# run-house/kubetorch

Hardware: NVIDIA H100
Metric: parallel_map_arg_plus_result_GBps (higher is better)
Workload: dtype f32

## Files before the change

kubetorch_b200/csrc/ktb_mlp.cu:

```cuda
#include "ktb_common.cuh"

#include <cuda.h>
#include <algorithm>
#include <atomic>
#include <climits>
#include <cmath>
#include <mutex>

namespace ktb {

constexpr int kMlpBlockM = 128;
constexpr int kMlpBlockK = 64;
constexpr int kMlpWgmmaK = 16;
constexpr int kMlpStages = 4;
constexpr int kMlpConsumers = 256;
constexpr int kMlpThreads = kMlpConsumers + 32;
int g_mlp_chunk_rows = 16896;

__device__ __forceinline__ void tma_load_2d(void* smem_dst, const CUtensorMap* map, int c0, int c1, uint64_t* bar) {
  asm volatile(
      "cp.async.bulk.tensor.2d.shared::cluster.global.mbarrier::complete_tx::bytes [%0], [%1, {%3, %4}], [%2];" ::
          "r"(smem_u32(smem_dst)),
      "l"(map), "r"(smem_u32(bar)), "r"(c0), "r"(c1)
      : "memory");
}
__device__ __forceinline__ void prefetch_tensormap(const CUtensorMap* map) {
  asm volatile("prefetch.tensormap [%0];" ::"l"(map) : "memory");
}
__device__ __forceinline__ void mbar_arrive(uint64_t* bar) {
  asm volatile("mbarrier.arrive.shared::cta.b64 _, [%0];" ::"r"(smem_u32(bar)) : "memory");
}
__device__ __forceinline__ void wgmma_fence() { asm volatile("wgmma.fence.sync.aligned;" ::: "memory"); }
__device__ __forceinline__ void wgmma_commit() { asm volatile("wgmma.commit_group.sync.aligned;" ::: "memory"); }
__device__ __forceinline__ void wgmma_wait_all() { asm volatile("wgmma.wait_group.sync.aligned 0;" ::: "memory"); }

__device__ __forceinline__ uint64_t make_smem_desc_sw128(const void* smem_tile) {
  const uint32_t addr = smem_u32(smem_tile);
  uint64_t d = 0;
  d |= (uint64_t)((addr & 0x3FFFFu) >> 4);
  d |= (uint64_t)1 << 16;
  d |= (uint64_t)(1024u >> 4) << 32;
  d |= (uint64_t)1 << 62;
  return d;
}

template <int N>
struct Wgmma;
template <>
struct Wgmma<256> {
  __device__ __forceinline__ static void mma(float (&d)[128], uint64_t adesc, uint64_t bdesc, uint32_t scale_d) {
    asm volatile(
        "{\n"
        ".reg .pred p;\n"
        "setp.ne.b32 p, %130, 0;\n"
        "wgmma.mma_async.sync.aligned.m64n256k16.f32.bf16.bf16 "
        "{%0,%1,%2,%3,%4,%5,%6,%7,%8,%9,%10,%11,%12,%13,%14,%15,%16,%17,%18,%19,%20,%21,%22,%23,%24,%25,%26,%27,%28,%29,%30,%31,%32,%33,%34,%35,%36,%37,%38,%39,%40,%41,%42,%43,%44,%45,%46,%47,%48,%49,%50,%51,%52,%53,%54,%55,%56,%57,%58,%59,%60,%61,%62,%63,%64,%65,%66,%67,%68,%69,%70,%71,%72,%73,%74,%75,%76,%77,%78,%79,%80,%81,%82,%83,%84,%85,%86,%87,%88,%89,%90,%91,%92,%93,%94,%95,%96,%97,%98,%99,%100,%101,%102,%103,%104,%105,%106,%107,%108,%109,%110,%111,%112,%113,%114,%115,%116,%117,%118,%119,%120,%121,%122,%123,%124,%125,%126,%127}, "
        "%128, %129, p, 1, 1, 0, 0;\n"
        "}\n"
        : "+f"(d[0]), "+f"(d[1]), "+f"(d[2]), "+f"(d[3]), "+f"(d[4]), "+f"(d[5]), "+f"(d[6]), "+f"(d[7]), "+f"(d[8]), "+f"(d[9]), "+f"(d[10]), "+f"(d[11]), "+f"(d[12]), "+f"(d[13]), "+f"(d[14]), "+f"(d[15]), "+f"(d[16]), "+f"(d[17]), "+f"(d[18]), "+f"(d[19]), "+f"(d[20]), "+f"(d[21]), "+f"(d[22]), "+f"(d[23]), "+f"(d[24]), "+f"(d[25]), "+f"(d[26]), "+f"(d[27]), "+f"(d[28]), "+f"(d[29]), "+f"(d[30]), "+f"(d[31]), "+f"(d[32]), "+f"(d[33]), "+f"(d[34]), "+f"(d[35]), "+f"(d[36]), "+f"(d[37]), "+f"(d[38]), "+f"(d[39]), "+f"(d[40]), "+f"(d[41]), "+f"(d[42]), "+f"(d[43]), "+f"(d[44]), "+f"(d[45]), "+f"(d[46]), "+f"(d[47]), "+f"(d[48]), "+f"(d[49]), "+f"(d[50]), "+f"(d[51]), "+f"(d[52]), "+f"(d[53]), "+f"(d[54]), "+f"(d[55]), "+f"(d[56]), "+f"(d[57]), "+f"(d[58]), "+f"(d[59]), "+f"(d[60]), "+f"(d[61]), "+f"(d[62]), "+f"(d[63]), "+f"(d[64]), "+f"(d[65]), "+f"(d[66]), "+f"(d[67]), "+f"(d[68]), "+f"(d[69]), "+f"(d[70]), "+f"(d[71]), "+f"(d[72]), "+f"(d[73]), "+f"(d[74]), "+f"(d[75]), "+f"(d[76]), "+f"(d[77]), "+f"(d[78]), "+f"(d[79]), "+f"(d[80]), "+f"(d[81]), "+f"(d[82]), "+f"(d[83]), "+f"(d[84]), "+f"(d[85]), "+f"(d[86]), "+f"(d[87]), "+f"(d[88]), "+f"(d[89]), "+f"(d[90]), "+f"(d[91]), "+f"(d[92]), "+f"(d[93]), "+f"(d[94]), "+f"(d[95]), "+f"(d[96]), "+f"(d[97]), "+f"(d[98]), "+f"(d[99]), "+f"(d[100]), "+f"(d[101]), "+f"(d[102]), "+f"(d[103]), "+f"(d[104]), "+f"(d[105]), "+f"(d[106]), "+f"(d[107]), "+f"(d[108]), "+f"(d[109]), "+f"(d[110]), "+f"(d[111]), "+f"(d[112]), "+f"(d[113]), "+f"(d[114]), "+f"(d[115]), "+f"(d[116]), "+f"(d[117]), "+f"(d[118]), "+f"(d[119]), "+f"(d[120]), "+f"(d[121]), "+f"(d[122]), "+f"(d[123]), "+f"(d[124]), "+f"(d[125]), "+f"(d[126]), "+f"(d[127])
        : "l"(adesc), "l"(bdesc), "r"(scale_d));
  }
};

template <>
struct Wgmma<128> {
  __device__ __forceinline__ static void mma(float (&d)[64], uint64_t adesc, uint64_t bdesc, uint32_t scale_d) {
    asm volatile(
        "{\n"
        ".reg .pred p;\n"
        "setp.ne.b32 p, %66, 0;\n"
        "wgmma.mma_async.sync.aligned.m64n128k16.f32.bf16.bf16 "
        "{%0,%1,%2,%3,%4,%5,%6,%7,%8,%9,%10,%11,%12,%13,%14,%15,%16,%17,%18,%19,%20,%21,%22,%23,%24,%25,%26,%27,%28,%29,%30,%31,%32,%33,%34,%35,%36,%37,%38,%39,%40,%41,%42,%43,%44,%45,%46,%47,%48,%49,%50,%51,%52,%53,%54,%55,%56,%57,%58,%59,%60,%61,%62,%63}, "
        "%64, %65, p, 1, 1, 0, 0;\n"
        "}\n"
        : "+f"(d[0]), "+f"(d[1]), "+f"(d[2]), "+f"(d[3]), "+f"(d[4]), "+f"(d[5]), "+f"(d[6]), "+f"(d[7]), "+f"(d[8]), "+f"(d[9]), "+f"(d[10]), "+f"(d[11]), "+f"(d[12]), "+f"(d[13]), "+f"(d[14]), "+f"(d[15]), "+f"(d[16]), "+f"(d[17]), "+f"(d[18]), "+f"(d[19]), "+f"(d[20]), "+f"(d[21]), "+f"(d[22]), "+f"(d[23]), "+f"(d[24]), "+f"(d[25]), "+f"(d[26]), "+f"(d[27]), "+f"(d[28]), "+f"(d[29]), "+f"(d[30]), "+f"(d[31]), "+f"(d[32]), "+f"(d[33]), "+f"(d[34]), "+f"(d[35]), "+f"(d[36]), "+f"(d[37]), "+f"(d[38]), "+f"(d[39]), "+f"(d[40]), "+f"(d[41]), "+f"(d[42]), "+f"(d[43]), "+f"(d[44]), "+f"(d[45]), "+f"(d[46]), "+f"(d[47]), "+f"(d[48]), "+f"(d[49]), "+f"(d[50]), "+f"(d[51]), "+f"(d[52]), "+f"(d[53]), "+f"(d[54]), "+f"(d[55]), "+f"(d[56]), "+f"(d[57]), "+f"(d[58]), "+f"(d[59]), "+f"(d[60]), "+f"(d[61]), "+f"(d[62]), "+f"(d[63])
        : "l"(adesc), "l"(bdesc), "r"(scale_d));
  }
};

template <>
struct Wgmma<64> {
  __device__ __forceinline__ static void mma(float (&d)[32], uint64_t adesc, uint64_t bdesc, uint32_t scale_d) {
    asm volatile(
        "{\n"
        ".reg .pred p;\n"
        "setp.ne.b32 p, %34, 0;\n"
        "wgmma.mma_async.sync.aligned.m64n64k16.f32.bf16.bf16 "
        "{%0,%1,%2,%3,%4,%5,%6,%7,%8,%9,%10,%11,%12,%13,%14,%15,%16,%17,%18,%19,%20,%21,%22,%23,%24,%25,%26,%27,%28,%29,%30,%31}, "
        "%32, %33, p, 1, 1, 0, 0;\n"
        "}\n"
        : "+f"(d[0]), "+f"(d[1]), "+f"(d[2]), "+f"(d[3]), "+f"(d[4]), "+f"(d[5]), "+f"(d[6]), "+f"(d[7]), "+f"(d[8]), "+f"(d[9]), "+f"(d[10]), "+f"(d[11]), "+f"(d[12]), "+f"(d[13]), "+f"(d[14]), "+f"(d[15]), "+f"(d[16]), "+f"(d[17]), "+f"(d[18]), "+f"(d[19]), "+f"(d[20]), "+f"(d[21]), "+f"(d[22]), "+f"(d[23]), "+f"(d[24]), "+f"(d[25]), "+f"(d[26]), "+f"(d[27]), "+f"(d[28]), "+f"(d[29]), "+f"(d[30]), "+f"(d[31])
        : "l"(adesc), "l"(bdesc), "r"(scale_d));
  }
};
template <int BLOCK_N, int STAGES>
struct MlpSmem {
  static constexpr int kABytes = kMlpBlockM * kMlpBlockK * 2;
  static constexpr int kBBytes = BLOCK_N * kMlpBlockK * 2;
  static constexpr int kStageBytes = kABytes + kBBytes;
  static constexpr int kBarrierOff = STAGES * kStageBytes;
  static constexpr int kTotal = kBarrierOff + 2 * STAGES * 8 + 1024 ;
};

template <int BLOCK_N, int STAGES>
__device__ __forceinline__ bool mlp_tile_mainloop(const CUtensorMap* map_a, const CUtensorMap* map_b, int K, int m0,
                                                  int n0, float (&acc)[BLOCK_N / 2]) {
  using S = MlpSmem<BLOCK_N, STAGES>;
  extern __shared__ uint8_t smem_raw[];
  uint8_t* smem = reinterpret_cast<uint8_t*>((reinterpret_cast<uintptr_t>(smem_raw) + 1023) & ~(uintptr_t)1023);
  uint64_t* full = reinterpret_cast<uint64_t*>(smem + S::kBarrierOff);
  uint64_t* empty = full + STAGES;

  const int warp = threadIdx.x >> 5;
  const int lane = threadIdx.x & 31;
  const int num_kb = K / kMlpBlockK;

  if (threadIdx.x == 0) {
#pragma unroll
    for (int s = 0; s < STAGES; ++s) {
      mbar_init(&full[s], 1);
      mbar_init(&empty[s], kMlpConsumers);
    }
    fence_barrier_init();
  }
  __syncthreads();

  if (warp == kMlpConsumers / 32) {
    if (lane == 0) {
      prefetch_tensormap(map_a);
      prefetch_tensormap(map_b);
      for (int kb = 0; kb < num_kb; ++kb) {
        const int s = kb % STAGES;
        mbar_wait(&empty[s], ((kb / STAGES) & 1) ^ 1);
        uint8_t* a_dst = smem + (size_t)s * S::kStageBytes;
        mbar_expect_tx(&full[s], S::kStageBytes);
        tma_load_2d(a_dst, map_a, kb * kMlpBlockK, m0, &full[s]);
        tma_load_2d(a_dst + S::kABytes, map_b, kb * kMlpBlockK, n0, &full[s]);
      }
    }
    return false;
  }

  const int wg = warp >> 2;
#pragma unroll
  for (int i = 0; i < BLOCK_N / 2; ++i) acc[i] = 0.f;
  for (int kb = 0; kb < num_kb; ++kb) {
    const int s = kb % STAGES;
    mbar_wait(&full[s], (kb / STAGES) & 1);
    const uint8_t* a_src = smem + (size_t)s * S::kStageBytes + wg * 64 * 128;
    const uint64_t adesc = make_smem_desc_sw128(a_src);
    const uint64_t bdesc = make_smem_desc_sw128(smem + (size_t)s * S::kStageBytes + S::kABytes);
    wgmma_fence();
#pragma unroll
    for (int k = 0; k < kMlpBlockK / kMlpWgmmaK; ++k) {
      Wgmma<BLOCK_N>::mma(acc, adesc + (uint64_t)(2 * k), bdesc + (uint64_t)(2 * k), (uint32_t)((kb | k) != 0));
    }
    wgmma_commit();
    wgmma_wait_all();
    mbar_arrive(&empty[s]);
  }
  return true;
}

__device__ __forceinline__ bool argmax_before(float v, int col, float best, int best_col) {
  const bool v_nan = v != v, best_nan = best != best;
  if (v_nan || best_nan) return v_nan && (!best_nan || col < best_col);
  return v > best || (v == best && col < best_col);
}

__device__ __forceinline__ uint4 philox4x32_10(uint4 c, uint2 k) {
#pragma unroll
  for (int i = 0; i < 10; ++i) {
    const uint32_t hi0 = __umulhi(0xD2511F53u, c.x), lo0 = 0xD2511F53u * c.x;
    const uint32_t hi1 = __umulhi(0xCD9E8D57u, c.z), lo1 = 0xCD9E8D57u * c.z;
    c = make_uint4(hi1 ^ c.y ^ k.x, lo1, hi0 ^ c.w ^ k.y, lo0);
    k.x += 0x9E3779B9u;
    k.y += 0xBB67AE85u;
  }
  return c;
}

__device__ __forceinline__ float gumbel_of(uint32_t x) {
  const float u = (float)(2u * (x >> 9) + 1u) * 5.9604644775390625e-8f;
  return -logf(-logf(u));
}

__device__ __forceinline__ void layer_pair(float a0, float a1, float a2, float a3, const __nv_bfloat16* bias, int col,
                                           int n_valid, int relu, __nv_bfloat162& y0, __nv_bfloat162& y1) {
  float v[4] = {a0, a1, a2, a3};
  if (bias != nullptr) {
#pragma unroll
    for (int c = 0; c < 2; ++c) {
      if (col + c < n_valid) {
        const float b = __bfloat162float(bias[col + c]);
        v[c] += b;
        v[2 + c] += b;
      }
    }
  }
  if (relu) {
#pragma unroll
    for (int q = 0; q < 4; ++q) v[q] = fmaxf(v[q], 0.f);
  }
  y0 = __floats2bfloat162_rn(v[0], v[1]);
  y1 = __floats2bfloat162_rn(v[2], v[3]);
}

template <int BLOCK_N>
__device__ __forceinline__ void sample_epilogue(const float (&acc)[BLOCK_N / 2], const __nv_bfloat16* bias, int col0,
                                                int n_valid, int relu, int row, bool st0, bool st1, int64_t* actions,
                                                float* log_probs, uint64_t seed, uint64_t row_base) {
  float mx[2] = {-INFINITY, -INFINITY};
  __nv_bfloat162 y[BLOCK_N / 4];
#pragma unroll
  for (int j = 0; j < BLOCK_N / 8; ++j) {
    const int col = col0 + 8 * j;
    if (col >= n_valid) continue;
    layer_pair(acc[4 * j], acc[4 * j + 1], acc[4 * j + 2], acc[4 * j + 3], bias, col, n_valid, relu, y[2 * j],
               y[2 * j + 1]);
#pragma unroll
    for (int q = 0; q < 4; ++q) {
      const float v = q & 1 ? __high2float(y[2 * j + (q >> 1)]) : __low2float(y[2 * j + (q >> 1)]);
      if (col + (q & 1) < n_valid && v > mx[q >> 1]) mx[q >> 1] = v;
    }
  }
#pragma unroll
  for (int h = 0; h < 2; ++h) {
#pragma unroll
    for (int m = 1; m <= 2; m <<= 1) {
      const float o = __shfl_xor_sync(0xffffffffu, mx[h], m);
      if (o > mx[h]) mx[h] = o;
    }
  }
  const uint2 key = make_uint2((uint32_t)seed, (uint32_t)(seed >> 32));
  float best[2] = {-INFINITY, -INFINITY}, best_y[2] = {0.f, 0.f}, sum[2] = {0.f, 0.f};
  int best_col[2] = {INT_MAX, INT_MAX};
#pragma unroll
  for (int j = 0; j < BLOCK_N / 8; ++j) {
    const int col = col0 + 8 * j;
    if (col >= n_valid) continue;
#pragma unroll
    for (int h = 0; h < 2; ++h) {
      const uint64_t i = row_base + (uint64_t)(row + 8 * h);
      const uint4 x = philox4x32_10(make_uint4((uint32_t)i, (uint32_t)(i >> 32), (uint32_t)col >> 1, 0u), key);
#pragma unroll
      for (int c = 0; c < 2; ++c) {
        if (col + c >= n_valid) continue;
        const float v = c ? __high2float(y[2 * j + h]) : __low2float(y[2 * j + h]);
        const float s = v + gumbel_of(c ? x.y : x.x);
        if (argmax_before(s, col + c, best[h], best_col[h])) {
          best[h] = s;
          best_col[h] = col + c;
          best_y[h] = v;
        }
        sum[h] += v == mx[h] ? 1.f : expf(v - mx[h]);
      }
    }
  }
#pragma unroll
  for (int h = 0; h < 2; ++h) {
#pragma unroll
    for (int m = 1; m <= 2; m <<= 1) {
      const float ov = __shfl_xor_sync(0xffffffffu, best[h], m);
      const int oc = __shfl_xor_sync(0xffffffffu, best_col[h], m);
      const float oy = __shfl_xor_sync(0xffffffffu, best_y[h], m);
      sum[h] += __shfl_xor_sync(0xffffffffu, sum[h], m);
      if (argmax_before(ov, oc, best[h], best_col[h])) {
        best[h] = ov;
        best_col[h] = oc;
        best_y[h] = oy;
      }
    }
  }
  if ((threadIdx.x & 3) == 0) {
    if (st0) {
      actions[row] = best_col[0];
      log_probs[row] = best_y[0] - mx[0] - logf(sum[0]);
    }
    if (st1) {
      actions[row + 8] = best_col[1];
      log_probs[row + 8] = best_y[1] - mx[1] - logf(sum[1]);
    }
  }
}

template <int BLOCK_N, int STAGES>
__device__ __forceinline__ void gaussian_epilogue(const float (&acc)[BLOCK_N / 2], const __nv_bfloat16* bias, int col0,
                                                  int n_valid, int relu, int row, bool st0, bool st1,
                                                  const float* log_std, float* actions, float* log_probs,
                                                  uint64_t seed, uint64_t row_base) {
  asm volatile("" : "+l"(seed), "+l"(row_base), "+l"(bias), "+r"(col0), "+r"(n_valid), "+r"(row));
  using S = MlpSmem<BLOCK_N, STAGES>;
  static_assert(BLOCK_N / 64 <= STAGES, "each warp's bf16 pairs fill its 16 A rows of BLOCK_N / 64 stages");
  extern __shared__ uint8_t smem_raw[];
  uint8_t* smem = reinterpret_cast<uint8_t*>((reinterpret_cast<uintptr_t>(smem_raw) + 1023) & ~(uintptr_t)1023);
  uint8_t* mine = smem + (threadIdx.x >> 5) * 16 * 128 + (threadIdx.x & 31) * 4;
  auto slot = [&](int w) { return reinterpret_cast<__nv_bfloat162*>(mine + (w >> 4) * S::kStageBytes + (w & 15) * 128); };
#pragma unroll
  for (int j = 0; j < BLOCK_N / 8; ++j) {
    const int col = col0 + 8 * j;
    if (col >= n_valid) continue;
    layer_pair(acc[4 * j], acc[4 * j + 1], acc[4 * j + 2], acc[4 * j + 3], bias, col, n_valid, relu, *slot(2 * j),
               *slot(2 * j + 1));
  }
  const uint2 key = make_uint2((uint32_t)seed, (uint32_t)(seed >> 32));
  const bool pairs = (n_valid & 1) == 0 && ((uintptr_t)actions & 7) == 0;
  float sum[2] = {0.f, 0.f};
#pragma unroll 1
  for (int j = 0; j < BLOCK_N / 8; ++j) {
    const int col = col0 + 8 * j;
    if (col >= n_valid) break;
    const __nv_bfloat162 y[2] = {*slot(2 * j), *slot(2 * j + 1)};
    const bool has1 = col + 1 < n_valid;
    const float ls[2] = {log_std[col], has1 ? log_std[col + 1] : 0.f};
    const float sg[2] = {expf(ls[0]), expf(ls[1])};
#pragma unroll
    for (int h = 0; h < 2; ++h) {
      const uint64_t i = row_base + (uint64_t)(row + 8 * h);
      const uint4 x = philox4x32_10(make_uint4((uint32_t)i, (uint32_t)(i >> 32), (uint32_t)col >> 1, 1u), key);
      float a[2];
#pragma unroll
      for (int c = 0; c < 2; ++c) {
        const float u = (float)(2u * ((c ? x.y : x.x) >> 9) + 1u) * 5.9604644775390625e-8f;
        const float z = normcdfinvf(u);
        a[c] = __fadd_rn(c ? __high2float(y[h]) : __low2float(y[h]), __fmul_rn(sg[c], z));
        if (c == 0 || has1) sum[h] += 0.5f * z * z + ls[c];
      }
      if (!(h ? st1 : st0)) continue;
      float* p = actions + (size_t)(row + 8 * h) * n_valid + col;
      if (pairs) {
        *reinterpret_cast<float2*>(p) = make_float2(a[0], a[1]);
      } else {
        p[0] = a[0];
        if (has1) p[1] = a[1];
      }
    }
  }
#pragma unroll
  for (int h = 0; h < 2; ++h) {
#pragma unroll
    for (int m = 1; m <= 2; m <<= 1) sum[h] += __shfl_xor_sync(0xffffffffu, sum[h], m);
  }
  if ((threadIdx.x & 3) == 0) {
    const float c = (float)n_valid * 0.918938533204672742f;
    if (st0) log_probs[row] = -sum[0] - c;
    if (st1) log_probs[row + 8] = -sum[1] - c;
  }
}

template <int BLOCK_N, int STAGES>
__global__ void __launch_bounds__(kMlpThreads, 1)
    mlp_layer_wgmma_kernel(const __grid_constant__ CUtensorMap map_a, const __grid_constant__ CUtensorMap map_b,
                           const __nv_bfloat16* __restrict__ bias, __nv_bfloat16* __restrict__ C,
                           int64_t* __restrict__ actions, float* __restrict__ log_probs, uint64_t seed,
                           uint64_t row_base, const float* __restrict__ log_std, float* __restrict__ gauss_actions,
                           int ldc, int n_valid, int K, int rows, int relu) {
  const int n0 = blockIdx.x * BLOCK_N;
  const int m0 = blockIdx.y * kMlpBlockM;
  const int lane = threadIdx.x & 31;
  const int col0 = n0 + 2 * (lane & 3);
  float acc[BLOCK_N / 2];
  if (!mlp_tile_mainloop<BLOCK_N, STAGES>(&map_a, &map_b, K, m0, n0, acc)) return;
  const int warp = threadIdx.x >> 5;
  const int wg = warp >> 2;

  const int row = m0 + wg * 64 + (warp & 3) * 16 + (lane >> 2);
  const bool st0 = row < rows, st1 = row + 8 < rows;
  if (log_std != nullptr) {
    gaussian_epilogue<BLOCK_N, STAGES>(acc, bias, col0, n_valid, relu, row, st0, st1, log_std, gauss_actions,
                                       log_probs, seed, row_base);
    return;
  }
  if (log_probs != nullptr) {
    sample_epilogue<BLOCK_N>(acc, bias, col0, n_valid, relu, row, st0, st1, actions, log_probs, seed, row_base);
    return;
  }
  const bool pairs = C != nullptr && (ldc & 1) == 0 && ((uintptr_t)C & 3) == 0;
  if (pairs && actions == nullptr && n0 + BLOCK_N <= n_valid) {
    __nv_bfloat16* p0 = C + (size_t)row * ldc + col0;
    __nv_bfloat16* p1 = p0 + (size_t)8 * ldc;
#pragma unroll
    for (int j = 0; j < BLOCK_N / 8; ++j) {
      __nv_bfloat162 y0, y1;
      layer_pair(acc[4 * j], acc[4 * j + 1], acc[4 * j + 2], acc[4 * j + 3], bias, col0 + 8 * j, n_valid, relu, y0, y1);
      if (st0) *reinterpret_cast<__nv_bfloat162*>(p0 + 8 * j) = y0;
      if (st1) *reinterpret_cast<__nv_bfloat162*>(p1 + 8 * j) = y1;
    }
    return;
  }
  float best[2] = {-INFINITY, -INFINITY};
  int best_col[2] = {INT_MAX, INT_MAX};
#pragma unroll
  for (int j = 0; j < BLOCK_N / 8; ++j) {
    const int col = col0 + 8 * j;
    __nv_bfloat162 y0, y1;
    layer_pair(acc[4 * j], acc[4 * j + 1], acc[4 * j + 2], acc[4 * j + 3], bias, col, n_valid, relu, y0, y1);
    if (C != nullptr) {
      __nv_bfloat16* p0 = C + (size_t)row * ldc + col;
      __nv_bfloat16* p1 = p0 + (size_t)8 * ldc;
      if (pairs && col + 1 < n_valid) {
        if (st0) *reinterpret_cast<__nv_bfloat162*>(p0) = y0;
        if (st1) *reinterpret_cast<__nv_bfloat162*>(p1) = y1;
      } else {
        if (st0 && col < n_valid) p0[0] = y0.x;
        if (st1 && col < n_valid) p1[0] = y1.x;
        if (st0 && col + 1 < n_valid) p0[1] = y0.y;
        if (st1 && col + 1 < n_valid) p1[1] = y1.y;
      }
    }
    if (actions != nullptr) {
      const float r[4] = {__low2float(y0), __high2float(y0), __low2float(y1), __high2float(y1)};
#pragma unroll
      for (int q = 0; q < 4; ++q) {
        const int h = q >> 1, c = col + (q & 1);
        if (c < n_valid && argmax_before(r[q], c, best[h], best_col[h])) {
          best[h] = r[q];
          best_col[h] = c;
        }
      }
    }
  }
  if (actions != nullptr) {
#pragma unroll
    for (int h = 0; h < 2; ++h) {
#pragma unroll
      for (int m = 1; m <= 2; m <<= 1) {
        const float ov = __shfl_xor_sync(0xffffffffu, best[h], m);
        const int oc = __shfl_xor_sync(0xffffffffu, best_col[h], m);
        if (argmax_before(ov, oc, best[h], best_col[h])) {
          best[h] = ov;
          best_col[h] = oc;
        }
      }
    }
    if ((lane & 3) == 0) {
      if (st0) actions[row] = best_col[0];
      if (st1) actions[row + 8] = best_col[1];
    }
  }
}

typedef CUresult (*PFN_tensorMapEncodeTiled)(CUtensorMap*, CUtensorMapDataType, cuuint32_t, void*, const cuuint64_t*,
                                             const cuuint64_t*, const cuuint32_t*, const cuuint32_t*,
                                             CUtensorMapInterleave, CUtensorMapSwizzle, CUtensorMapL2promotion,
                                             CUtensorMapFloatOOBfill);
static PFN_tensorMapEncodeTiled g_encode = nullptr;
static std::once_flag g_encode_once;

static int get_encoder() {
  std::call_once(g_encode_once, [] {
    void* fn = nullptr;
    cudaDriverEntryPointQueryResult qres;
    if (cudaGetDriverEntryPoint("cuTensorMapEncodeTiled", &fn, cudaEnableDefault, &qres) == cudaSuccess &&
        qres == cudaDriverEntryPointSuccess)
      g_encode = reinterpret_cast<PFN_tensorMapEncodeTiled>(fn);
  });
  KTB_REQUIRE(g_encode != nullptr, KTB_ERR_CUDA, "cuTensorMapEncodeTiled is not available from the driver");
  return KTB_OK;
}

static int encode_map(CUtensorMap* map, const void* base, uint64_t rows, uint64_t cols, uint32_t box_rows);

static int make_map(CUtensorMap* map, const void* base, uint64_t rows, uint64_t cols, uint32_t box_rows) {
  struct Key {
    const void* base;
    uint64_t rows, cols;
    uint32_t box;
    bool operator==(const Key& o) const { return base == o.base && rows == o.rows && cols == o.cols && box == o.box; }
  };
  struct Slot {
    Key key;
    CUtensorMap map;
    bool used = false;
  };
  constexpr int kSlots = 64;
  thread_local Slot cache[kSlots];
  const Key k{base, rows, cols, box_rows};
  const size_t h = ((uintptr_t)base >> 8) * 0x9E3779B97F4A7C15ull + rows * 31 + cols * 7 + box_rows;
  Slot& s = cache[h % kSlots];
  if (s.used && s.key == k) {
    *map = s.map;
    return KTB_OK;
  }
  int rc = encode_map(map, base, rows, cols, box_rows);
  if (rc) return rc;
  s.key = k;
  s.map = *map;
  s.used = true;
  return KTB_OK;
}

static int encode_map(CUtensorMap* map, const void* base, uint64_t rows, uint64_t cols, uint32_t box_rows) {
  cuuint64_t gdim[2] = {cols, rows};
  cuuint64_t gstride[1] = {cols * 2};
  cuuint32_t box[2] = {(cuuint32_t)kMlpBlockK, box_rows};
  cuuint32_t estr[2] = {1, 1};
  CUresult r = g_encode(map, CU_TENSOR_MAP_DATA_TYPE_BFLOAT16, 2, const_cast<void*>(base), gdim, gstride, box, estr,
                        CU_TENSOR_MAP_INTERLEAVE_NONE, CU_TENSOR_MAP_SWIZZLE_128B, CU_TENSOR_MAP_L2_PROMOTION_L2_256B,
                        CU_TENSOR_MAP_FLOAT_OOB_FILL_NONE);
  KTB_REQUIRE(r == CUDA_SUCCESS, KTB_ERR_CUDA, "cuTensorMapEncodeTiled failed with CUresult %d", (int)r);
  return KTB_OK;
}

template <typename KernelT>
static int ensure_smem_attr(KernelT kfn, int smem_bytes, std::atomic<unsigned>& done_mask, int dev) {
  if (dev >= 0 && dev < 32 && (done_mask.load(std::memory_order_acquire) & (1u << dev))) return KTB_OK;
  cudaError_t e = cudaFuncSetAttribute(kfn, cudaFuncAttributeMaxDynamicSharedMemorySize, smem_bytes);
  if (e != cudaSuccess) {
    set_error("cudaFuncSetAttribute(max dynamic shared memory = %d) failed: %s", smem_bytes, cudaGetErrorString(e));
    return KTB_ERR_CUDA;
  }
  if (dev >= 0 && dev < 32) done_mask.fetch_or(1u << dev, std::memory_order_release);
  return KTB_OK;
}

template <int BLOCK_N>
static int launch_layer(int dev, const void* A, const void* B, const void* bias, void* C, int64_t* actions,
                        float* log_probs, uint64_t seed, uint64_t row_base, const float* log_std, float* gauss_actions,
                        size_t M, int N, int K, int ldc, bool relu, cudaStream_t stream) {
  using S = MlpSmem<BLOCK_N, kMlpStages>;
  static_assert(S::kTotal <= 232448, "the TMA ring must fit the 227 KiB a block may own");
  CUtensorMap ma, mb;
  int rc = make_map(&ma, A, M, (uint64_t)K, kMlpBlockM);
  if (rc) return rc;
  rc = make_map(&mb, B, (uint64_t)N, (uint64_t)K, BLOCK_N);
  if (rc) return rc;
  auto kfn = mlp_layer_wgmma_kernel<BLOCK_N, kMlpStages>;
  static std::atomic<unsigned> attr_done{0};
  rc = ensure_smem_attr(kfn, S::kTotal, attr_done, dev);
  if (rc) return rc;
  dim3 grid((unsigned)((N + BLOCK_N - 1) / BLOCK_N), (unsigned)((M + kMlpBlockM - 1) / kMlpBlockM));
  kfn<<<grid, kMlpThreads, S::kTotal, stream>>>(ma, mb, static_cast<const __nv_bfloat16*>(bias),
                                                static_cast<__nv_bfloat16*>(C), actions, log_probs, seed, row_base,
                                                log_std, gauss_actions, ldc, N, K, (int)M, relu);
  KTB_CK(cudaGetLastError());
  return KTB_OK;
}

struct MlpParams {
  const void *W1, *b1, *W2, *b2, *W3, *b3;
  void* logits;
  int64_t* actions;
  float* log_probs = nullptr;
  uint64_t seed = 0, row_base = 0;
  const float* log_std = nullptr;
  float* gauss_actions = nullptr;
};

static int mlp_hidden(int dev, const void* A, const void* W, const void* b, void* H, size_t rows, int d_hidden, int K,
                      cudaStream_t st) {
  return launch_layer<256>(dev, A, W, b, H, nullptr, nullptr, 0, 0, nullptr, nullptr, rows, d_hidden, K, d_hidden,
                           true, st);
}

static int mlp_head(int dev, const MlpParams& p, const void* h2, size_t r0, size_t rows, int d_hidden, int d_out,
                    cudaStream_t st) {
  void* y = p.logits ? static_cast<__nv_bfloat16*>(p.logits) + r0 * d_out : nullptr;
  int64_t* act = p.actions ? p.actions + r0 : nullptr;
  float* lp = p.log_probs ? p.log_probs + r0 : nullptr;
  float* ga = p.gauss_actions ? p.gauss_actions + r0 * d_out : nullptr;
  const uint64_t rb = p.row_base + r0;
  if (d_out <= 64)
    return launch_layer<64>(dev, h2, p.W3, p.b3, y, act, lp, p.seed, rb, p.log_std, ga, rows, d_out, d_hidden, d_out,
                            false, st);
  if (d_out <= 128)
    return launch_layer<128>(dev, h2, p.W3, p.b3, y, act, lp, p.seed, rb, p.log_std, ga, rows, d_out, d_hidden, d_out,
                             false, st);
  return launch_layer<256>(dev, h2, p.W3, p.b3, y, act, lp, p.seed, rb, p.log_std, ga, rows, d_out, d_hidden, d_out,
                           false, st);
}

static int mlp_check(const char* fn, size_t M, int d_in, int d_hidden, int d_out, const MlpParams& p, const void* obs,
                     const void* scratch, const void* stage) {
  KTB_REQUIRE(d_in > 0 && d_in % kMlpBlockK == 0, KTB_ERR_ARG, "%s: d_in=%d must be a multiple of 64", fn, d_in);
  KTB_REQUIRE(d_hidden > 0 && d_hidden % 256 == 0, KTB_ERR_ARG, "%s: d_hidden=%d must be a multiple of 256", fn,
              d_hidden);
  if (M > 0) {
    KTB_REQUIRE(p.logits || p.actions || p.log_std, KTB_ERR_ARG, "%s: logits and actions are both null", fn);
    if (p.log_std) {
      KTB_REQUIRE(p.gauss_actions && p.log_probs && !p.logits && !p.actions, KTB_ERR_ARG,
                  "%s: the Gaussian head needs fp32 actions and log_probs, and stores nothing else", fn);
      KTB_REQUIRE((((uintptr_t)p.log_std | (uintptr_t)p.gauss_actions) & 3) == 0, KTB_ERR_ARG,
                  "%s: log_std and actions must be 4-byte aligned", fn);
    }
    KTB_REQUIRE(d_out >= 1, KTB_ERR_ARG, "%s: d_out=%d must be positive", fn, d_out);
    KTB_REQUIRE(d_out <= 256, KTB_ERR_UNSUPPORTED, "%s: d_out=%d (heads up to 256 wide)", fn, d_out);
    KTB_REQUIRE((((uintptr_t)p.logits | (uintptr_t)p.b1 | (uintptr_t)p.b2 | (uintptr_t)p.b3) & 1) == 0, KTB_ERR_ARG,
                "%s: logits and biases must be 2-byte aligned", fn);
    KTB_REQUIRE(((uintptr_t)p.actions & 7) == 0, KTB_ERR_ARG, "%s: actions must be 8-byte aligned", fn);
    KTB_REQUIRE(((uintptr_t)p.log_probs & 3) == 0, KTB_ERR_ARG, "%s: log_probs must be 4-byte aligned", fn);
  }
  KTB_REQUIRE((((uintptr_t)obs | (uintptr_t)p.W1 | (uintptr_t)p.W2 | (uintptr_t)p.W3 | (uintptr_t)scratch |
                (uintptr_t)stage) & 15) == 0,
              KTB_ERR_ARG, "%s: obs, weights, scratch and stage must be 16-byte aligned", fn);
  return KTB_OK;
}
}

using namespace ktb;

extern "C" {

size_t ktb_mlp_scratch_bytes(size_t M, int d_hidden) {
  const size_t rows = std::min<size_t>(M, (size_t)g_mlp_chunk_rows);
  return 2 * rows * (size_t)d_hidden * 2;
}

size_t ktb_mlp_stage_bytes(size_t M, int d_in) {
  const size_t rows = std::min<size_t>(M, (size_t)g_mlp_chunk_rows);
  return 2 * rows * (size_t)d_in * 2;
}

int g_mlp_stage_ce = 0;

static int mlp_run(const char* fn, int dev, const void* obs, size_t M, int d_in, int d_hidden, int d_out,
                   const MlpParams& p, void* scratch, void* stage, uintptr_t stream) {
  int rc = require_device(dev);
  if (rc) return rc;
  if (M == 0) return KTB_OK;
  KTB_REQUIRE(obs && p.W1 && p.W2 && p.W3 && scratch, KTB_ERR_ARG, "%s: null argument", fn);
  rc = mlp_check(fn, M, d_in, d_hidden, d_out, p, obs, scratch, stage);
  if (rc) return rc;
  KTB_REQUIRE(g_mlp_chunk_rows % kMlpBlockM == 0 && g_mlp_chunk_rows > 0, KTB_ERR_ARG, "%s: bad chunk rows", fn);
  rc = get_encoder();
  if (rc) return rc;
  KTB_GUARD(dev);
  DeviceInfo* di = device_info(dev);
  cudaStream_t st = reinterpret_cast<cudaStream_t>(stream);
  cudaStream_t side = di->stream_exec;
  const size_t chunk = std::min<size_t>(M, (size_t)g_mlp_chunk_rows);
  __nv_bfloat16* h1 = static_cast<__nv_bfloat16*>(scratch);
  __nv_bfloat16* h2 = h1 + chunk * (size_t)d_hidden;
  const __nv_bfloat16* x = static_cast<const __nv_bfloat16*>(obs);
  __nv_bfloat16* stg = static_cast<__nv_bfloat16*>(stage);
  const MapParams ident = make_params(1, 0);
  cudaEvent_t evs[5] = {nullptr, nullptr, nullptr, nullptr, nullptr};
  struct EvGuard {
    cudaEvent_t* e;
    ~EvGuard() {
      for (int i = 0; i < 5; ++i)
        if (e[i]) cudaEventDestroy(e[i]);
    }
  } ev_guard{evs};
  static std::mutex side_mu[kMaxDevices];
  std::unique_lock<std::mutex> side_lock;
  if (stg) {
    side_lock = std::unique_lock<std::mutex>(side_mu[dev]);
    for (int i = 0; i < 5; ++i) KTB_CK(cudaEventCreateWithFlags(&evs[i], cudaEventDisableTiming));
    KTB_CK(cudaEventRecord(evs[0], st));
    KTB_CK(cudaStreamWaitEvent(side, evs[0], 0));
  }
  size_t c = 0;
  for (size_t r0 = 0; r0 < M; r0 += chunk, ++c) {
    const size_t rows = std::min(chunk, M - r0);
    const __nv_bfloat16* a1 = x + r0 * d_in;
    if (stg) {
      const int b = (int)(c & 1);
      __nv_bfloat16* dstb = stg + (size_t)b * chunk * d_in;
      if (c >= 2) KTB_CK(cudaStreamWaitEvent(side, evs[3 + b], 0));
      if (g_mlp_stage_ce) {
        KTB_CK(cudaMemcpyAsync(dstb, a1, rows * (size_t)d_in * 2, cudaMemcpyDefault, side));
      } else {
        rc = launch_map(dev, KTB_OP_IDENTITY, KTB_U8, a1, dstb, rows * (size_t)d_in * 2, ident, KTB_VARIANT_AUTO, side);
        if (rc) return rc;
      }
      KTB_CK(cudaEventRecord(evs[1 + b], side));
      KTB_CK(cudaStreamWaitEvent(st, evs[1 + b], 0));
      a1 = dstb;
    }
    rc = mlp_hidden(dev, a1, p.W1, p.b1, h1, rows, d_hidden, d_in, st);
    if (rc) return rc;
    if (stg) KTB_CK(cudaEventRecord(evs[3 + (int)(c & 1)], st));
    rc = mlp_hidden(dev, h1, p.W2, p.b2, h2, rows, d_hidden, d_hidden, st);
    if (rc) return rc;
    rc = mlp_head(dev, p, h2, r0, rows, d_hidden, d_out, st);
    if (rc) return rc;
  }
  return KTB_OK;
}

namespace ktb {
__global__ void mlp_wait_ready_kernel(const unsigned long long* ready, unsigned long long seq, unsigned int* status) {
  if (threadIdx.x == 0) (void)spin_until(ready, seq, status);
}
__global__ void mlp_ack_kernel(unsigned long long* ack, unsigned long long seq) {
  if (threadIdx.x == 0) {
    __threadfence_system();
    st_release_sys(ack, seq);
  }
}
}

static int mlp_pushed_run(const char* fn, int dev, const void* stage_local, size_t stage_stride, size_t M, int d_in,
                          int d_hidden, int d_out, const MlpParams& p, void* scratch, void* ctrl_local,
                          void* ctrl_root_peer, int rank, size_t chunk_rows, unsigned long long seq, uintptr_t stream) {
  int rc = require_device(dev);
  if (rc) return rc;
  KTB_REQUIRE(stage_local && ctrl_local && ctrl_root_peer && p.W1 && p.W2 && p.W3 && scratch, KTB_ERR_ARG,
              "%s: null argument", fn);
  KTB_REQUIRE(rank >= 0 && rank < 16 && seq > 0, KTB_ERR_ARG, "%s: bad rank/seq", fn);
  KTB_REQUIRE(M % kMlpBlockM == 0, KTB_ERR_ARG, "%s: M=%zu must be a multiple of %d", fn, M, kMlpBlockM);
  KTB_REQUIRE(chunk_rows > 0 && chunk_rows % kMlpBlockM == 0, KTB_ERR_ARG,
              "%s: chunk_rows=%zu must be a positive multiple of %d", fn, chunk_rows, kMlpBlockM);
  rc = mlp_check(fn, M, d_in, d_hidden, d_out, p, stage_local, scratch, nullptr);
  if (rc) return rc;
  const size_t n_chunks = (M + chunk_rows - 1) / chunk_rows;
  KTB_REQUIRE(n_chunks <= KTB_PUSH_MAX_CHUNKS, KTB_ERR_ARG, "%s: %zu chunks exceed %d", fn, n_chunks,
              KTB_PUSH_MAX_CHUNKS);
  KTB_REQUIRE(M * (size_t)d_in * 2 <= stage_stride, KTB_ERR_ARG, "%s: shard exceeds stage_stride", fn);
  rc = get_encoder();
  if (rc) return rc;
  KTB_GUARD(dev);
  cudaStream_t st = reinterpret_cast<cudaStream_t>(stream);
  uint8_t* cl = static_cast<uint8_t*>(ctrl_local);
  const unsigned long long* ready = reinterpret_cast<const unsigned long long*>(cl + KTB_CTRL_READY);
  unsigned int* status = reinterpret_cast<unsigned int*>(cl + KTB_CTRL_STATUS);
  unsigned long long* ack =
      reinterpret_cast<unsigned long long*>(static_cast<uint8_t*>(ctrl_root_peer) + KTB_CTRL_ACK) + rank;
  const __nv_bfloat16* x =
      reinterpret_cast<const __nv_bfloat16*>(static_cast<const uint8_t*>(stage_local) + (size_t)(seq & 1) * stage_stride);
  __nv_bfloat16* h1 = static_cast<__nv_bfloat16*>(scratch);
  __nv_bfloat16* h2 = h1 + std::min(chunk_rows, M) * (size_t)d_hidden;
  size_t c = 0;
  for (size_t r0 = 0; r0 < M; r0 += chunk_rows, ++c) {
    const size_t rows = std::min(chunk_rows, M - r0);
    mlp_wait_ready_kernel<<<1, 32, 0, st>>>(ready + c, seq, status);
    KTB_CK(cudaGetLastError());
    const __nv_bfloat16* a1 = x + r0 * d_in;
    rc = mlp_hidden(dev, a1, p.W1, p.b1, h1, rows, d_hidden, d_in, st);
    if (rc) return rc;
    rc = mlp_hidden(dev, h1, p.W2, p.b2, h2, rows, d_hidden, d_hidden, st);
    if (rc) return rc;
    rc = mlp_head(dev, p, h2, r0, rows, d_hidden, d_out, st);
    if (rc) return rc;
  }
  mlp_ack_kernel<<<1, 32, 0, st>>>(ack, seq);
  KTB_CK(cudaGetLastError());
  return KTB_OK;
}

int ktb_mlp_bf16_pushed(int dev, const void* stage_local, size_t stage_stride, size_t M, int d_in, int d_hidden, int d_out,
                        const void* W1, const void* W2, const void* W3, void* logits, void* scratch, void* ctrl_local,
                        void* ctrl_root_peer, int rank, size_t chunk_rows, unsigned long long seq, uintptr_t stream) {
  const char* fn = "ktb_mlp_bf16_pushed";
  int rc = require_device(dev);
  if (rc) return rc;
  KTB_REQUIRE(logits || M == 0, KTB_ERR_ARG, "%s: null argument", fn);
  KTB_REQUIRE(d_out == 64, KTB_ERR_UNSUPPORTED, "%s: d_out=%d (the 64-wide head)", fn, d_out);
  const MlpParams p{W1, nullptr, W2, nullptr, W3, nullptr, logits, nullptr};
  return mlp_pushed_run(fn, dev, stage_local, stage_stride, M, d_in, d_hidden, d_out, p, scratch, ctrl_local,
                        ctrl_root_peer, rank, chunk_rows, seq, stream);
}

int ktb_mlp_bf16_policy_pushed(int dev, const void* stage_local, size_t stage_stride, size_t M, int d_in, int d_hidden,
                               int d_out, const void* W1, const void* b1, const void* W2, const void* b2,
                               const void* W3, const void* b3, void* logits, int64_t* actions, void* scratch,
                               void* ctrl_local, void* ctrl_root_peer, int rank, size_t chunk_rows,
                               unsigned long long seq, uintptr_t stream) {
  const MlpParams p{W1, b1, W2, b2, W3, b3, logits, actions};
  return mlp_pushed_run("ktb_mlp_bf16_policy_pushed", dev, stage_local, stage_stride, M, d_in, d_hidden, d_out, p,
                        scratch, ctrl_local, ctrl_root_peer, rank, chunk_rows, seq, stream);
}

static int mlp_run_64(const char* fn, int dev, const void* obs, size_t M, int d_in, int d_hidden, int d_out,
                      const void* W1, const void* W2, const void* W3, void* logits, void* scratch, void* stage,
                      uintptr_t stream) {
  int rc = require_device(dev);
  if (rc || M == 0) return rc;
  KTB_REQUIRE(logits, KTB_ERR_ARG, "%s: null argument", fn);
  KTB_REQUIRE(d_out == 64, KTB_ERR_UNSUPPORTED, "%s: d_out=%d (the 64-wide head)", fn, d_out);
  KTB_REQUIRE(((uintptr_t)logits & 15) == 0, KTB_ERR_ARG, "%s: logits must be 16-byte aligned", fn);
  const MlpParams p{W1, nullptr, W2, nullptr, W3, nullptr, logits, nullptr};
  return mlp_run(fn, dev, obs, M, d_in, d_hidden, d_out, p, scratch, stage, stream);
}

int ktb_mlp_bf16(int dev, const void* obs, size_t M, int d_in, int d_hidden, int d_out, const void* W1,
                 const void* W2, const void* W3, void* logits, void* scratch, uintptr_t stream) {
  return mlp_run_64("ktb_mlp_bf16", dev, obs, M, d_in, d_hidden, d_out, W1, W2, W3, logits, scratch, nullptr, stream);
}

int ktb_mlp_bf16_staged(int dev, const void* obs_peer, size_t M, int d_in, int d_hidden, int d_out, const void* W1,
                        const void* W2, const void* W3, void* logits, void* scratch, void* stage, uintptr_t stream) {
  KTB_REQUIRE(stage, KTB_ERR_ARG, "ktb_mlp_bf16_staged: null stage buffer");
  return mlp_run_64("ktb_mlp_bf16_staged", dev, obs_peer, M, d_in, d_hidden, d_out, W1, W2, W3, logits, scratch, stage,
                    stream);
}

int ktb_mlp_bf16_policy(int dev, const void* obs, size_t M, int d_in, int d_hidden, int d_out, const void* W1,
                        const void* b1, const void* W2, const void* b2, const void* W3, const void* b3, void* logits,
                        int64_t* actions, void* scratch, void* stage, uintptr_t stream) {
  const MlpParams p{W1, b1, W2, b2, W3, b3, logits, actions};
  return mlp_run("ktb_mlp_bf16_policy", dev, obs, M, d_in, d_hidden, d_out, p, scratch, stage, stream);
}

int ktb_mlp_bf16_policy_sample(int dev, const void* obs, size_t M, int d_in, int d_hidden, int d_out, const void* W1,
                               const void* b1, const void* W2, const void* b2, const void* W3, const void* b3,
                               uint64_t seed, uint64_t row_base, int64_t* actions, float* log_probs, void* scratch,
                               void* stage, uintptr_t stream) {
  const char* fn = "ktb_mlp_bf16_policy_sample";
  int rc = require_device(dev);
  if (rc) return rc;
  KTB_REQUIRE(M == 0 || (actions && log_probs), KTB_ERR_ARG, "%s: actions and log_probs are required", fn);
  const MlpParams p{W1, b1, W2, b2, W3, b3, nullptr, actions, log_probs, seed, row_base};
  return mlp_run(fn, dev, obs, M, d_in, d_hidden, d_out, p, scratch, stage, stream);
}

int ktb_mlp_bf16_policy_sample_pushed(int dev, const void* stage_local, size_t stage_stride, size_t M, int d_in,
                                      int d_hidden, int d_out, const void* W1, const void* b1, const void* W2,
                                      const void* b2, const void* W3, const void* b3, uint64_t seed, uint64_t row_base,
                                      int64_t* actions, float* log_probs, void* scratch, void* ctrl_local,
                                      void* ctrl_root_peer, int rank, size_t chunk_rows, unsigned long long seq,
                                      uintptr_t stream) {
  const char* fn = "ktb_mlp_bf16_policy_sample_pushed";
  int rc = require_device(dev);
  if (rc) return rc;
  KTB_REQUIRE(M == 0 || (actions && log_probs), KTB_ERR_ARG, "%s: actions and log_probs are required", fn);
  const MlpParams p{W1, b1, W2, b2, W3, b3, nullptr, actions, log_probs, seed, row_base};
  return mlp_pushed_run(fn, dev, stage_local, stage_stride, M, d_in, d_hidden, d_out, p, scratch, ctrl_local,
                        ctrl_root_peer, rank, chunk_rows, seq, stream);
}

int ktb_mlp_bf16_policy_gaussian(int dev, const void* obs, size_t M, int d_in, int d_hidden, int d_out, const void* W1,
                                 const void* b1, const void* W2, const void* b2, const void* W3, const void* b3,
                                 const float* log_std, uint64_t seed, uint64_t row_base, float* actions,
                                 float* log_probs, void* scratch, void* stage, uintptr_t stream) {
  const char* fn = "ktb_mlp_bf16_policy_gaussian";
  int rc = require_device(dev);
  if (rc) return rc;
  KTB_REQUIRE(M == 0 || (log_std && actions && log_probs), KTB_ERR_ARG,
              "%s: log_std, actions and log_probs are required", fn);
  const MlpParams p{W1, b1, W2, b2, W3, b3, nullptr, nullptr, log_probs, seed, row_base, log_std, actions};
  return mlp_run(fn, dev, obs, M, d_in, d_hidden, d_out, p, scratch, stage, stream);
}

int ktb_mlp_bf16_policy_gaussian_pushed(int dev, const void* stage_local, size_t stage_stride, size_t M, int d_in,
                                        int d_hidden, int d_out, const void* W1, const void* b1, const void* W2,
                                        const void* b2, const void* W3, const void* b3, const float* log_std,
                                        uint64_t seed, uint64_t row_base, float* actions, float* log_probs,
                                        void* scratch, void* ctrl_local, void* ctrl_root_peer, int rank,
                                        size_t chunk_rows, unsigned long long seq, uintptr_t stream) {
  const char* fn = "ktb_mlp_bf16_policy_gaussian_pushed";
  int rc = require_device(dev);
  if (rc) return rc;
  KTB_REQUIRE(M == 0 || (log_std && actions && log_probs), KTB_ERR_ARG,
              "%s: log_std, actions and log_probs are required", fn);
  const MlpParams p{W1, b1, W2, b2, W3, b3, nullptr, nullptr, log_probs, seed, row_base, log_std, actions};
  return mlp_pushed_run(fn, dev, stage_local, stage_stride, M, d_in, d_hidden, d_out, p, scratch, ctrl_local,
                        ctrl_root_peer, rank, chunk_rows, seq, stream);
}

}
```

Before: 2970.

## Enable programmatic dependent launch for MLP layers and prefetch weights before grid wait

Each MLP layer kernel is now launched with programmatic stream serialization and calls griddepcontrol.launch_dependents right after barrier init. The next layer can therefore start its prologue while the previous one drains. The producer issues TMA loads of the weight tiles for the first pipeline stages before griddepcontrol.wait, and loads only the activation tiles after the dependency resolves. This hides launch latency and weight-load latency between the chained layers, at the cost of more complex producer logic and a reliance on weights not being written by the preceding kernel.

```diff
diff --git a/kubetorch_b200/csrc/ktb_mlp.cu b/kubetorch_b200/csrc/ktb_mlp.cu
--- a/kubetorch_b200/csrc/ktb_mlp.cu
+++ b/kubetorch_b200/csrc/ktb_mlp.cu
@@ -33,6 +33,10 @@
 __device__ __forceinline__ void wgmma_fence() { asm volatile("wgmma.fence.sync.aligned;" ::: "memory"); }
 __device__ __forceinline__ void wgmma_commit() { asm volatile("wgmma.commit_group.sync.aligned;" ::: "memory"); }
 __device__ __forceinline__ void wgmma_wait_all() { asm volatile("wgmma.wait_group.sync.aligned 0;" ::: "memory"); }
+__device__ __forceinline__ void griddep_launch_dependents() {
+  asm volatile("griddepcontrol.launch_dependents;" ::: "memory");
+}
+__device__ __forceinline__ void griddep_wait() { asm volatile("griddepcontrol.wait;" ::: "memory"); }
 
 __device__ __forceinline__ uint64_t make_smem_desc_sw128(const void* smem_tile) {
   const uint32_t addr = smem_u32(smem_tile);
@@ -124,22 +128,34 @@
     fence_barrier_init();
   }
   __syncthreads();
+  griddep_launch_dependents();
 
   if (warp == kMlpConsumers / 32) {
     if (lane == 0) {
       prefetch_tensormap(map_a);
       prefetch_tensormap(map_b);
+      const int pre = num_kb < STAGES ? num_kb : STAGES;
+      for (int kb = 0; kb < pre; ++kb) {
+        mbar_expect_tx(&full[kb], S::kStageBytes);
+        tma_load_2d(smem + (size_t)kb * S::kStageBytes + S::kABytes, map_b, kb * kMlpBlockK, n0, &full[kb]);
+      }
+      griddep_wait();
       for (int kb = 0; kb < num_kb; ++kb) {
         const int s = kb % STAGES;
-        mbar_wait(&empty[s], ((kb / STAGES) & 1) ^ 1);
         uint8_t* a_dst = smem + (size_t)s * S::kStageBytes;
-        mbar_expect_tx(&full[s], S::kStageBytes);
+        if (kb >= pre) {
+          mbar_wait(&empty[s], ((kb / STAGES) & 1) ^ 1);
+          mbar_expect_tx(&full[s], S::kStageBytes);
+          tma_load_2d(a_dst + S::kABytes, map_b, kb * kMlpBlockK, n0, &full[s]);
+        }
         tma_load_2d(a_dst, map_a, kb * kMlpBlockK, m0, &full[s]);
-        tma_load_2d(a_dst + S::kABytes, map_b, kb * kMlpBlockK, n0, &full[s]);
-      }
+      }
+    } else {
+      griddep_wait();
     }
     return false;
   }
+  griddep_wait();
 
   const int wg = warp >> 2;
 #pragma unroll
@@ -530,10 +546,19 @@
   rc = ensure_smem_attr(kfn, S::kTotal, attr_done, dev);
   if (rc) return rc;
   dim3 grid((unsigned)((N + BLOCK_N - 1) / BLOCK_N), (unsigned)((M + kMlpBlockM - 1) / kMlpBlockM));
-  kfn<<<grid, kMlpThreads, S::kTotal, stream>>>(ma, mb, static_cast<const __nv_bfloat16*>(bias),
-                                                static_cast<__nv_bfloat16*>(C), actions, log_probs, seed, row_base,
-                                                log_std, gauss_actions, ldc, N, K, (int)M, relu);
-  KTB_CK(cudaGetLastError());
+  cudaLaunchAttribute attr[1];
+  attr[0].id = cudaLaunchAttributeProgrammaticStreamSerialization;
+  attr[0].val.programmaticStreamSerializationAllowed = 1;
+  cudaLaunchConfig_t cfg = {};
+  cfg.gridDim = grid;
+  cfg.blockDim = dim3(kMlpThreads);
+  cfg.dynamicSmemBytes = S::kTotal;
+  cfg.stream = stream;
+  cfg.attrs = attr;
+  cfg.numAttrs = 1;
+  KTB_CK(cudaLaunchKernelEx(&cfg, kfn, ma, mb, static_cast<const __nv_bfloat16*>(bias),
+                            static_cast<__nv_bfloat16*>(C), actions, log_probs, seed, row_base, log_std, gauss_actions,
+                            ldc, N, K, (int)M, (int)relu));
   return KTB_OK;
 }
 
```

Measured after the change: 2965, median of 6. About the same (-0.2%).
